# randyjhc/vit-colmap

Hardware: AMD Instinct MI355X
Metric: images/sec extracted + pair-matches/sec (N×D brute-force NN) (higher is better)
Workload: dtype bf16 (ViT) / u8+i32 (matcher); 1 GPU; configs[1]+configs[2]: DINOv2 ViT-S/14 extract of 50 640x480 images (512 keypoints, 384-D uint8 descriptors) then exhaustive mutual-NN + ratio matching of all pairs among the extracted images; images_total=50, images_rank0=50, num_keypoints=512, descriptor_dim=384, parallelism=images+pairs sharded x1

## Files before the change

vit_colmap_amd/csrc/gemm.hip:

```cpp
#include <hip/hip_runtime.h>
#include <stdint.h>

#include "../../include/vitcolmap_hip.h"
#include "common.h"
#include "device.h"

namespace {

typedef __bf16 v8bf __attribute__((ext_vector_type(8)));
typedef __bf16 v4bf __attribute__((ext_vector_type(4)));
typedef float v4f __attribute__((ext_vector_type(4)));

constexpr int BM = 128;
constexpr int BN = 128;
constexpr int BK = 64;
constexpr int kImg = 128 * 128;
constexpr int kStage = 2 * kImg;

enum { EPI_BIAS = 0, EPI_GELU = 1, EPI_RESIDUAL = 2, EPI_PATCH = 3, EPI_SWIGLU = 4 };
static_assert(EPI_BIAS == VC_EPI_BIAS && EPI_GELU == VC_EPI_GELU && EPI_RESIDUAL == VC_EPI_RESIDUAL && EPI_SWIGLU == VC_EPI_SWIGLU,
              "epilogue codes of the ABI");

__device__ __forceinline__ float gelu_erf(float x) {
  const float ax = __builtin_fabsf(x);
// ... 520 lines not shown
        const int row = 8 * p + prow;
        *(v4u*)(tp + row * 128 + (((lane & 7) ^ ((row >> 1) & 7)) << 4)) = *(const v4u*)&xf[4 * c + p];
      }
#pragma unroll
      for (int k4 = 0; k4 < 4; ++k4)
        xf[4 * c + k4] = *(const v8bf*)(tp + r * 128 + (((2 * k4 + h) ^ fsw) << 4));
    }
    if (LN) {
      auto expand = [](uint32_t u) { return (v2f){__uint_as_float(u << 16), __uint_as_float(u & 0xffff0000u)}; };
      v2f s2 = {0.f, 0.f};
#pragma unroll
      for (int ks = 0; ks < XKS; ++ks) {
        const v4u u = *(const v4u*)&xf[ks];
#pragma unroll
        for (int j = 0; j < 4; ++j) s2 += expand(u[j]);
      }
      float sum = s2[0] + s2[1];
      sum += __shfl_xor(sum, 32);
      const float mean = sum * (1.0f / XK);
      const v2f mean2 = {mean, mean};
#pragma unroll
      for (int ks = 0; ks < XKS; ++ks) asm volatile("" : "+v"(xf[ks]));
      v2f q2 = {0.f, 0.f};
#pragma unroll
      for (int ks = 0; ks < XKS; ++ks) {
        const v4u u = *(const v4u*)&xf[ks];
#pragma unroll
        for (int j = 0; j < 4; ++j) { const v2f d = expand(u[j]) - mean2; q2 = __builtin_elementwise_fma(d, d, q2); }
      }
      float q = q2[0] + q2[1];
      q += __shfl_xor(q, 32);
      const float rstd = __builtin_amdgcn_rsqf(q * (1.0f / XK) + eps);
      const v2f rstd2 = {rstd, rstd};
#pragma unroll
      for (int ks = 0; ks < XKS; ++ks) asm volatile("" : "+v"(xf[ks]));
#pragma unroll
      for (int ks = 0; ks < XKS; ++ks) {
        const v4u u = *(const v4u*)&xf[ks];
#pragma unroll
        for (int j = 0; j < 4; ++j) {
          const v2f y = (expand(u[j]) - mean2) * rstd2;
          xf[ks][2 * j] = (__bf16)y[0];
          xf[ks][2 * j + 1] = (__bf16)y[1];
        }
      }
    }
  };

  const __amdgpu_buffer_rsrc_t out_rs = __builtin_amdgcn_make_buffer_rsrc(out, 0, (int)((size_t)M * N * 2), 0x00020000);
  uint8_t* const tr_out = lds + XOffStage + wave * (2 * XChunk);
  uint8_t* const tr_res = tr_out + 2048;
  const int crow = lane >> 2, cch = lane & 3;
  const int rsw = (r >> 2) & 3;
  v4u resq[2];
  auto load_res = [&](int m_base, int nb) {
    if (EPI == EPI_RESIDUAL) {
#pragma unroll
      for (int q = 0; q < 2; ++q)
        resq[q] = *(const v4u*)(res + (size_t)min(m_base + crow + 16 * q, M - 1) * N + nb * 32 + cch * 8);
    }
  };
  v16f pa;
  float ev[16];
  uint32_t ep[8];
  v4u eo[2];
  int pm_base = 0, pnb = 0;
  auto res_to_lds = [&]() {
    if (EPI == EPI_RESIDUAL) {
#pragma unroll
      for (int q = 0; q < 2; ++q) {
        const int row = crow + 16 * q;
        *(v4u*)(tr_res + row * 64 + ((cch ^ ((row >> 2) & 3)) << 4)) = resq[q];
      }
    }
  };
  uint32_t gq[8];
  uint32_t gres[8];
  uint32_t gbad = 0;
  auto slice = [&](int sl) {
    if (EPI == EPI_GELU && GT) {
      typedef __bf16 v2bf __attribute__((ext_vector_type(2)));
      if (sl < 4) {
        const int g = sl;
        const v2bf lo = {(__bf16)pa[4 * g], (__bf16)pa[4 * g + 1]}, hi = {(__bf16)pa[4 * g + 2], (__bf16)pa[4 * g + 3]};
        ep[2 * g] = *(const uint32_t*)&lo;
        ep[2 * g + 1] = *(const uint32_t*)&hi;
        if (sl == 0) gbad = 0;
      }
      if (sl >= 4 && sl < 12) {
        const int qd = sl - 4;
        const uint32_t b0 = ep[qd] & 0xffffu, b1 = ep[qd] >> 16;
        const uint32_t k0 = (b0 & 0x7fffu) - kGtLo, k1 = (b1 & 0x7fffu) - kGtLo;
        gbad = max(gbad, max(k0, k1));
        const uint32_t a0 = min(k0, kGtN - 1) * 4 + ((b0 >> 15) << 1), a1 = min(k1, kGtN - 1) * 4 + ((b1 >> 15) << 1);
        gq[2 * (qd & 3)] = *(const uint16_t*)(gt_l + a0);
        gq[2 * (qd & 3) + 1] = *(const uint16_t*)(gt_l + a1);
      }
      if (sl >= 7 && sl < 15) {
        const int qd = sl - 7;
        gres[qd] = gq[2 * (qd & 3)] | (gq[2 * (qd & 3) + 1] << 16);
      }
      if (sl == 15) {
        if (__any(gbad >= kGtN)) {
#pragma unroll
          for (int qd = 0; qd < 8; ++qd) {
            const v2f_t xin = {__uint_as_float(ep[qd] << 16), __uint_as_float(ep[qd] & 0xffff0000u)};
            const v2f_t y = gelu_erf2(xin);
            const v2bf o = {(__bf16)y[0], (__bf16)y[1]};
            ep[qd] = *(const uint32_t*)&o;
          }
        } else {
#pragma unroll
          for (int qd = 0; qd < 8; ++qd) ep[qd] = gres[qd];
        }
      }
      if (sl == 16) {
#pragma unroll
        for (int i = 0; i < 4; ++i) {
          const auto sw = __builtin_amdgcn_permlane32_swap(ep[i], ep[i + 4], false, false);
          ep[i] = sw[0];
          ep[i + 4] = sw[1];
        }
      }
      if (sl == 17) {
        *(v4u*)(tr_out + r * 64 + (((2 * h) ^ rsw) << 4)) = (v4u){ep[0], ep[1], ep[4], ep[5]};
        *(v4u*)(tr_out + r * 64 + (((2 * h + 1) ^ rsw) << 4)) = (v4u){ep[2], ep[3], ep[6], ep[7]};
      }
      if (sl == 19) {
#pragma unroll
        for (int q = 0; q < 2; ++q) {
          const int row = crow + 16 * q;
          eo[q] = *(const v4u*)(tr_out + row * 64 + ((cch ^ ((row >> 2) & 3)) << 4));
        }
      }
      if (sl == 22) {
#pragma unroll
        for (int q = 0; q < 2; ++q) {
          const int row = crow + 16 * q;
          __builtin_amdgcn_raw_buffer_store_b128(eo[q], out_rs, (int)(((size_t)(pm_base + row) * N + pnb * 32 + cch * 8) * 2), 0, 0);
        }
      }
      return;
    }
    if (sl < 8) {
      const int j0 = 2 * sl;
      if (EPI == EPI_GELU) {
        const v2f_t y = gelu_erf2((v2f_t){pa[j0], pa[j0 + 1]});
        ev[j0] = y[0];
        ev[j0 + 1] = y[1];
      } else if (EPI == EPI_RESIDUAL) {
        if ((sl & 1) == 0) {
          const int g = sl >> 1;
          const v4bf rv = *(const v4bf*)(tr_res + r * 64 + ((g ^ rsw) << 4) + 8 * h);
#pragma unroll
          for (int j = 0; j < 4; ++j) ev[4 * g + j] = pa[4 * g + j] + (float)rv[j];
        }
      } else {
        ev[j0] = pa[j0];
        ev[j0 + 1] = pa[j0 + 1];
      }
    } else if (sl < 12) {
      const int g = sl - 8;
      typedef __bf16 v2bf __attribute__((ext_vector_type(2)));
      const v2bf lo = {(__bf16)ev[4 * g], (__bf16)ev[4 * g + 1]}, hi = {(__bf16)ev[4 * g + 2], (__bf16)ev[4 * g + 3]};
      ep[2 * g] = *(const uint32_t*)&lo;
      ep[2 * g + 1] = *(const uint32_t*)&hi;
    } else if (sl == 12) {
#pragma unroll
      for (int i = 0; i < 4; ++i) {
        const auto sw = __builtin_amdgcn_permlane32_swap(ep[i], ep[i + 4], false, false);
        ep[i] = sw[0];
        ep[i + 4] = sw[1];
      }
    } else if (sl == 13) {
      *(v4u*)(tr_out + r * 64 + (((2 * h) ^ rsw) << 4)) = (v4u){ep[0], ep[1], ep[4], ep[5]};
      *(v4u*)(tr_out + r * 64 + (((2 * h + 1) ^ rsw) << 4)) = (v4u){ep[2], ep[3], ep[6], ep[7]};
    } else if (sl == 15) {
#pragma unroll
      for (int q = 0; q < 2; ++q) {
        const int row = crow + 16 * q;
        eo[q] = *(const v4u*)(tr_out + row * 64 + ((cch ^ ((row >> 2) & 3)) << 4));
      }
    } else if (sl == 19) {
#pragma unroll
      for (int q = 0; q < 2; ++q) {
        const int row = crow + 16 * q;
        __builtin_amdgcn_raw_buffer_store_b128(eo[q], out_rs, (int)(((size_t)(pm_base + row) * N + pnb * 32 + cch * 8) * 2), 0, 0);
      }
    }
  };

  v16f acc;
  int mt_cur = -1, slot = 0;
  int mt = s0 / n_nb, nb = s0 - mt * n_nb;
  for (int i = 0; i < n; ++i) {
    if (i >= 2) {
      if (EPI == EPI_RESIDUAL) asm volatile("s_waitcnt vmcnt(7)" ::: "memory");
      else asm volatile("s_waitcnt vmcnt(5)" ::: "memory");
    } else {
      asm volatile("s_waitcnt vmcnt(3)" ::: "memory");
    }
    asm volatile("s_waitcnt lgkmcnt(0)\n\ts_barrier" ::: "memory");
    const bool pending = i > 0;
    if (pending) res_to_lds();
    const bool reload = mt != mt_cur;
    const int m_base = mt * XRows + wave * 32;
    if (reload) {
      x_issue(mt);
      if (pending) {
#pragma unroll
        for (int sl = 0; sl < XKS; ++sl) slice(sl);
      }
      x_finish();
      mt_cur = mt;
    }
    load_res(m_base, nb);
    const uint8_t* st = lds + slot * XStage + lane * 16;
    {
      const float* bl = bias_l + nb * 32 + 4 * h;
#pragma unroll
      for (int g = 0; g < 4; ++g) {
        const v4f bv = *(const v4f*)(bl + 8 * g);
#pragma unroll
        for (int j = 0; j < 4; ++j) acc[4 * g + j] = bv[j];
      }
    }
    {
      constexpr int XRD = (EPI == EPI_GELU && GT) ? 6 : XReadAhead;
      v8bf wf[XKS];
#pragma unroll
      for (int ks = 0; ks < XRD; ++ks) wf[ks] = *(const v8bf*)(st + ks * 1024);
      __builtin_amdgcn_sched_barrier(0);
      if (pending && !reload) {
#pragma unroll
        for (int ks = 0; ks < XKS; ++ks) {
          acc = __builtin_amdgcn_mfma_f32_32x32x16_bf16(wf[ks], xf[ks], acc, 0, 0, 0);
          if (ks + XRD < XKS) wf[ks + XRD] = *(const v8bf*)(st + (ks + XRD) * 1024);
          slice(ks);
          if (ks == XIssue0 || ks == XIssue0 + XIssueStep || ks == XIssue0 + 2 * XIssueStep)
            issue_piece((ks - XIssue0) / XIssueStep);
          __builtin_amdgcn_sched_barrier(0);
        }
      } else {
#pragma unroll
        for (int ks = 0; ks < XKS; ++ks) {
          acc = __builtin_amdgcn_mfma_f32_32x32x16_bf16(wf[ks], xf[ks], acc, 0, 0, 0);
          if (ks + XRD < XKS) wf[ks + XRD] = *(const v8bf*)(st + (ks + XRD) * 1024);
          if (ks == XIssue0 || ks == XIssue0 + XIssueStep || ks == XIssue0 + 2 * XIssueStep)
            issue_piece((ks - XIssue0) / XIssueStep);
          __builtin_amdgcn_sched_barrier(0);
        }
      }
    }
    pa = acc;
    pm_base = m_base;
    pnb = nb;
    slot = slot + 1 == XNS ? 0 : slot + 1;
    if (++nb == n_nb) { nb = 0; ++mt; }
  }
  res_to_lds();
#pragma unroll
  for (int sl = 0; sl < XKS; ++sl) slice(sl);
  asm volatile("s_waitcnt vmcnt(0)" ::: "memory");
}

__global__ __launch_bounds__(256) void xs_prepare_kernel(const float* __restrict__ W, const float* __restrict__ b,
                                                         const float* __restrict__ gamma, const float* __restrict__ beta,
                                                         int N, __bf16* __restrict__ Wp, float* __restrict__ biasf) {
  const int lane = threadIdx.x & 63;
  const int nfeat = blockIdx.x * 4 + (threadIdx.x >> 6);
  if (nfeat >= N) return;
  const int nb = nfeat >> 5, rr = nfeat & 31;
  float dot = 0.f;
  for (int k = lane; k < XK; k += 64) {
    const float w = W[(size_t)nfeat * XK + k];
    const float wg = gamma ? w * gamma[k] : w;
    if (beta) dot += w * beta[k];
    const int ks = k >> 4, hh = (k >> 3) & 1, j = k & 7;
    Wp[(((size_t)nb * XKS + ks) * 64 + hh * 32 + rr) * 8 + j] = (__bf16)wg;
  }
#pragma unroll
  for (int o = 32; o > 0; o >>= 1) dot += __shfl_xor(dot, o);
  if (lane == 0) biasf[nfeat] = (b ? b[nfeat] : 0.f) + dot;
}


constexpr int MStage = 2 * XStage;
constexpr int MNS = 2;

constexpr int M2OffB1 = MNS * MStage;
constexpr int M2OffGt = M2OffB1 + 1536 * 4;
constexpr int M2OffB2 = M2OffGt + 8704;
constexpr int M2OffTrA = M2OffB2 + 1536;
constexpr int M2OffTrB = M2OffTrA + 4 * XChunk;
constexpr int M2OffG = M2OffTrB + 4 * XChunk;
constexpr int M2Lds = M2OffG + 2 * 4 * 2048;
static_assert(M2Lds <= 160 * 1024, "fused MLP: LDS budget");

constexpr int M2ReadAhead = 6;
constexpr int M2PiecesA = 3;
constexpr int M2Issue0 = 1;
constexpr int M2IssueStep = 3;
constexpr int M2IssueStepB = 2;
__global__ __launch_bounds__(512, 2) void mlp2_kernel(__bf16* __restrict__ X, const uint8_t* __restrict__ Wm,
                                                      const float* __restrict__ b1f, const float* __restrict__ b2f,
                                                      int M, int n_chunks, int n_tiles, float eps,
                                                      const uint16_t* __restrict__ gelu_tab) {
  __shared__ __attribute__((aligned(1024))) uint8_t lds[M2Lds];
  const int tid = threadIdx.x, lane = tid & 63;
  const int wave = __builtin_amdgcn_readfirstlane(tid >> 6);
  const bool roleB = wave >= 4;
  const int pairw = wave & 3;
  const int r = lane & 31, h = lane >> 5;
  const int G = gridDim.x, bid = blockIdx.x;
  const int my_tiles = bid < n_tiles ? (n_tiles - bid + G - 1) / G : 0;
  const int n = my_tiles * n_chunks;
  if (n <= 0) return;

  float* const b1_l = (float*)(lds + M2OffB1);
  float* const b2_l = (float*)(lds + M2OffB2);
  uint8_t* const gt_l = lds + M2OffGt;
  for (int i = tid; i < n_chunks * 32; i += 512) b1_l[i] = b1f[i];
  for (int i = tid; i < XK; i += 512) b2_l[i] = b2f[i];
  for (int i = tid; i < kGtBytes / 4; i += 512) ((uint32_t*)gt_l)[i] = ((const uint32_t*)gelu_tab)[i];

  const uint32_t lds0 = vc::lds_addr(&lds[0]);
  const uint32_t lane_off = (uint32_t)lane * 16u;
  constexpr int NA = M2PiecesA, NB = 12 - NA;
  auto issue_piece = [&](int c1, int c2, int slot, int i) {
    const int role = wave >> 2, q = wave & 3;
    if (i >= (role ? NB : NA)) return;
    const int id = role ? 4 * NA + q * NB + i : q * NA + i;
    const int half = id >= 24, idx = id - 24 * half;
    const int c = half ? c2 : c1;
    const uint8_t* sbase = Wm + (size_t)c * MStage + (size_t)half * XStage + (size_t)idx * 1024;
    const uint32_t dst = lds0 + (uint32_t)slot * MStage + (uint32_t)half * XStage + (uint32_t)idx * 1024u;
    vc::lds_dma16(sbase, lane_off, dst);
  };
  auto issue = [&](int c1, int c2, int slot) {
#pragma unroll
    for (int i = 0; i < (NA > NB ? NA : NB); ++i) issue_piece(c1, c2, slot, i);
  };
  typedef __bf16 v2bf __attribute__((ext_vector_type(2)));
  typedef float v2f __attribute__((ext_vector_type(2)));

  int chunk = 0, slot = 0, tile = bid;
  auto chunk_of = [&](int j) { return j % n_chunks; };
  auto issue_stage = [&](int j, int slot_) {
    const int c1 = chunk_of(min(max(j, 0), n - 1)), c2 = chunk_of(min(max(j - 2, 0), n - 1));
    issue(c1, c2, slot_);
  };
  issue_stage(0, 0);
  if (!roleB) {
    v8bf xf[XKS];
    uint8_t* const tp = lds + M2OffTrA + pairw * XChunk;
    const int prow = lane >> 3;
    v16f hprev;
    uint32_t pb[8], gq[8], gres[8], gbad = 0;
    auto gelu_slice = [&](int sl, int parity) {
      if (sl < 4) {
        const int g = sl;
        const v2bf lo = {(__bf16)hprev[4 * g], (__bf16)hprev[4 * g + 1]}, hi = {(__bf16)hprev[4 * g + 2], (__bf16)hprev[4 * g + 3]};
        pb[2 * g] = *(const uint32_t*)&lo;
        pb[2 * g + 1] = *(const uint32_t*)&hi;
        if (sl == 0) gbad = 0;
      }
      if (sl >= 4 && sl < 12) {
        const int qd = sl - 4;
        const uint32_t b0 = pb[qd] & 0xffffu, b1 = pb[qd] >> 16;
        const uint32_t k0 = (b0 & 0x7fffu) - kGtLo, k1 = (b1 & 0x7fffu) - kGtLo;
        gbad = max(gbad, max(k0, k1));
        gq[2 * (qd & 3)] = *(const uint16_t*)(gt_l + min(k0, kGtN - 1) * 4 + ((b0 >> 15) << 1));
        gq[2 * (qd & 3) + 1] = *(const uint16_t*)(gt_l + min(k1, kGtN - 1) * 4 + ((b1 >> 15) << 1));
      }
      if (sl >= 7 && sl < 15) {
        const int qd = sl - 7;
        gres[qd] = gq[2 * (qd & 3)] | (gq[2 * (qd & 3) + 1] << 16);
      }
      if (sl == 15) {
        if (__any(gbad >= kGtN)) {
#pragma unroll
          for (int qd = 0; qd < 8; ++qd) {
            const v2f_t y = gelu_erf2((v2f_t){__uint_as_float(pb[qd] << 16), __uint_as_float(pb[qd] & 0xffff0000u)});
            const v2bf o = {(__bf16)y[0], (__bf16)y[1]};
            gres[qd] = *(const uint32_t*)&o;
          }
        }
      }
      if (sl == 16) {
        uint8_t* const gb = lds + M2OffG + (parity * 4 + pairw) * 2048 + lane * 16;
        *(v4u*)gb = (v4u){gres[0], gres[1], gres[2], gres[3]};
        *(v4u*)(gb + 1024) = (v4u){gres[4], gres[5], gres[6], gres[7]};
      }
    };
    for (int i = 0; i <= n + 1; ++i) {
      asm volatile("s_waitcnt vmcnt(0)" ::: "memory");
      asm volatile("s_waitcnt lgkmcnt(0)\n\ts_barrier" ::: "memory");
      const bool do_issue = i <= n;
      const int nc1 = chunk_of(min(max(i + 1, 0), n - 1)), nc2 = chunk_of(min(max(i - 1, 0), n - 1));
      if (do_issue && !(i < n && i > 0)) issue_stage(i + 1, slot ^ 1);
      if (i < n) {
        if (chunk == 0) {
          const int m0w = tile * 128 + pairw * 32;
#pragma unroll
          for (int p = 0; p < 4; ++p) {
            const int m = min(m0w + 8 * p + prow, M - 1);
            const uint8_t* src = (const uint8_t*)X + (size_t)m * (XK * 2) + (lane & 7) * 16;
#pragma unroll
            for (int c = 0; c < XK / 64; ++c) *(v4u*)&xf[4 * c + p] = *(const v4u*)(src + c * 128);
          }
          const int fsw = (r >> 1) & 7;
#pragma unroll
          for (int c = 0; c < XK / 64; ++c) {
#pragma unroll
            for (int p = 0; p < 4; ++p) {
              const int row = 8 * p + prow;
              *(v4u*)(tp + row * 128 + (((lane & 7) ^ ((row >> 1) & 7)) << 4)) = *(const v4u*)&xf[4 * c + p];
            }
#pragma unroll
            for (int k4 = 0; k4 < 4; ++k4)
              xf[4 * c + k4] = *(const v8bf*)(tp + r * 128 + (((2 * k4 + h) ^ fsw) << 4));
          }
          auto expand = [](uint32_t u) { return (v2f){__uint_as_float(u << 16), __uint_as_float(u & 0xffff0000u)}; };
          v2f s2 = {0.f, 0.f};
#pragma unroll
          for (int ks = 0; ks < XKS; ++ks) {
            const v4u u = *(const v4u*)&xf[ks];
#pragma unroll
            for (int j = 0; j < 4; ++j) s2 += expand(u[j]);
          }
          float sum = s2[0] + s2[1];
          sum += __shfl_xor(sum, 32);
          const float mean = sum * (1.0f / XK);
          const v2f mean2 = {mean, mean};
#pragma unroll
          for (int ks = 0; ks < XKS; ++ks) asm volatile("" : "+v"(xf[ks]));
          v2f q2 = {0.f, 0.f};
#pragma unroll
          for (int ks = 0; ks < XKS; ++ks) {
            const v4u u = *(const v4u*)&xf[ks];
#pragma unroll
            for (int j = 0; j < 4; ++j) { const v2f d = expand(u[j]) - mean2; q2 = __builtin_elementwise_fma(d, d, q2); }
          }
          float q = q2[0] + q2[1];
          q += __shfl_xor(q, 32);
          const float rstd = __builtin_amdgcn_rsqf(q * (1.0f / XK) + eps);
          const v2f rstd2 = {rstd, rstd};
#pragma unroll
          for (int ks = 0; ks < XKS; ++ks) asm volatile("" : "+v"(xf[ks]));
#pragma unroll
          for (int ks = 0; ks < XKS; ++ks) {
            const v4u u = *(const v4u*)&xf[ks];
#pragma unroll
            for (int j = 0; j < 4; ++j) {
              const v2f y = (expand(u[j]) - mean2) * rstd2;
              xf[ks][2 * j] = (__bf16)y[0];
              xf[ks][2 * j + 1] = (__bf16)y[1];
            }
          }
        }
        const uint8_t* st = lds + slot * MStage + lane * 16;
        v16f hacc;
        {
          const float* bl = b1_l + chunk * 32 + 4 * h;
#pragma unroll
          for (int g = 0; g < 4; ++g) {
            const v4f bv = *(const v4f*)(bl + 8 * g);
#pragma unroll
            for (int j = 0; j < 4; ++j) hacc[4 * g + j] = bv[j];
          }
        }
        {
          constexpr int RD = M2ReadAhead;
          v8bf wf[XKS];
#pragma unroll
          for (int ks = 0; ks < RD; ++ks) wf[ks] = *(const v8bf*)(st + ks * 1024);
          __builtin_amdgcn_sched_barrier(0);
          __builtin_amdgcn_s_setprio(1);
          if (i > 0) {
#pragma unroll
            for (int ks = 0; ks < XKS; ++ks) {
              hacc = __builtin_amdgcn_mfma_f32_32x32x16_bf16(wf[ks], xf[ks], hacc, 0, 0, 0);
              if (ks + RD < XKS) wf[ks + RD] = *(const v8bf*)(st + (ks + RD) * 1024);
              gelu_slice(ks, (i - 1) & 1);
              if (ks >= M2Issue0 && ks < M2Issue0 + NA * M2IssueStep && (ks - M2Issue0) % M2IssueStep == 0 && do_issue)
                issue_piece(nc1, nc2, slot ^ 1, (ks - M2Issue0) / M2IssueStep);
              __builtin_amdgcn_sched_barrier(0);
            }
          } else {
#pragma unroll
            for (int ks = 0; ks < XKS; ++ks) {
              hacc = __builtin_amdgcn_mfma_f32_32x32x16_bf16(wf[ks], xf[ks], hacc, 0, 0, 0);
              if (ks + RD < XKS) wf[ks + RD] = *(const v8bf*)(st + (ks + RD) * 1024);
              __builtin_amdgcn_sched_barrier(0);
            }
          }
        }
        __builtin_amdgcn_s_setprio(0);
        hprev = hacc;
        if (++chunk == n_chunks) { chunk = 0; tile += G; }
      } else if (i == n) {
#pragma unroll
        for (int sl = 0; sl < XKS; ++sl) gelu_slice(sl, (i - 1) & 1);
      }
      slot ^= 1;
    }
  } else {
    v16f oacc[12];
    const __amdgpu_buffer_rsrc_t out_rs = __builtin_amdgcn_make_buffer_rsrc(X, 0, (int)((size_t)M * XK * 2), 0x00020000);
    const int crow = lane >> 2, cch = lane & 3;
    const int rsw = (r >> 2) & 3;
    uint8_t* const tr_out = lds + M2OffTrB + pairw * XChunk;
    uint8_t* const tr_res = tr_out + 2048;
    int pchunk = 0;
    for (int i = 0; i <= n + 1; ++i) {
      asm volatile("s_waitcnt vmcnt(0)" ::: "memory");
      asm volatile("s_waitcnt lgkmcnt(0)\n\ts_barrier" ::: "memory");
      const bool do_issue = i <= n;
      const int nc1 = chunk_of(min(max(i + 1, 0), n - 1)), nc2 = chunk_of(min(max(i - 1, 0), n - 1));
      if (i >= 2) {
        if (pchunk == 0) {
#pragma unroll
          for (int ob = 0; ob < 12; ++ob)
#pragma unroll
            for (int j = 0; j < 16; ++j) oacc[ob][j] = 0.f;
        }
        const uint8_t* gb = lds + M2OffG + ((i & 1) * 4 + pairw) * 2048 + lane * 16;
        const v8bf g_s0 = *(const v8bf*)gb, g_s1 = *(const v8bf*)(gb + 1024);
        const uint8_t* st2 = lds + slot * MStage + XStage + lane * 16;
        {
          constexpr int RD = M2ReadAhead;
          v8bf wf[24];
#pragma unroll
          for (int q = 0; q < RD; ++q) wf[q] = *(const v8bf*)(st2 + q * 1024);
#pragma unroll
          for (int q = 0; q < 24; ++q) {
            oacc[q >> 1] = __builtin_amdgcn_mfma_f32_32x32x16_bf16(wf[q], (q & 1) ? g_s1 : g_s0, oacc[q >> 1], 0, 0, 0);
            if (q + RD < 24) wf[q + RD] = *(const v8bf*)(st2 + (q + RD) * 1024);
            constexpr int BSTEP = NB <= 6 ? M2IssueStep : M2IssueStepB;
            if (q >= M2Issue0 && q < M2Issue0 + NB * BSTEP && (q - M2Issue0) % BSTEP == 0 && do_issue)
              issue_piece(nc1, nc2, slot ^ 1, (q - M2Issue0) / BSTEP);
          }
        }
        if (pchunk == n_chunks - 1) {
          const int m0w = tile * 128 + pairw * 32;
#pragma unroll 1
          for (int ob = 0; ob < 12; ++ob) {
            v4u resq[2];
#pragma unroll
            for (int q = 0; q < 2; ++q)
              resq[q] = *(const v4u*)(X + (size_t)min(m0w + crow + 16 * q, M - 1) * XK + ob * 32 + cch * 8);
#pragma unroll
            for (int q = 0; q < 2; ++q) {
              const int row = crow + 16 * q;
              *(v4u*)(tr_res + row * 64 + ((cch ^ ((row >> 2) & 3)) << 4)) = resq[q];
            }
            v16f oa;
            switch (ob) {
#define VC_OB(k) case k: oa = oacc[k]; break;
              VC_OB(0) VC_OB(1) VC_OB(2) VC_OB(3) VC_OB(4) VC_OB(5) VC_OB(6) VC_OB(7) VC_OB(8) VC_OB(9) VC_OB(10)
              default: oa = oacc[11]; break;
#undef VC_OB
            }
            uint32_t ep[8];
#pragma unroll
            for (int g = 0; g < 4; ++g) {
              const v4bf rv = *(const v4bf*)(tr_res + r * 64 + ((g ^ rsw) << 4) + 8 * h);
              const v4f bv = *(const v4f*)(b2_l + ob * 32 + 8 * g + 4 * h);
              float v[4];
#pragma unroll
              for (int j = 0; j < 4; ++j) v[j] = oa[4 * g + j] + bv[j] + (float)rv[j];
              const v2bf lo = {(__bf16)v[0], (__bf16)v[1]}, hi = {(__bf16)v[2], (__bf16)v[3]};
              ep[2 * g] = *(const uint32_t*)&lo;
              ep[2 * g + 1] = *(const uint32_t*)&hi;
            }
#pragma unroll
            for (int k = 0; k < 4; ++k) {
              const auto sw = __builtin_amdgcn_permlane32_swap(ep[k], ep[k + 4], false, false);
              ep[k] = sw[0];
              ep[k + 4] = sw[1];
            }
            *(v4u*)(tr_out + r * 64 + (((2 * h) ^ rsw) << 4)) = (v4u){ep[0], ep[1], ep[4], ep[5]};
            *(v4u*)(tr_out + r * 64 + (((2 * h + 1) ^ rsw) << 4)) = (v4u){ep[2], ep[3], ep[6], ep[7]};
#pragma unroll
            for (int q = 0; q < 2; ++q) {
              const int row = crow + 16 * q;
              const v4u o = *(const v4u*)(tr_out + row * 64 + ((cch ^ ((row >> 2) & 3)) << 4));
              __builtin_amdgcn_raw_buffer_store_b128(o, out_rs, (int)(((size_t)(m0w + row) * XK + ob * 32 + cch * 8) * 2), 0, 0);
            }
          }
          tile += G;
        }
        if (++pchunk == n_chunks) pchunk = 0;
      }
      if (do_issue && i < 2) issue_stage(i + 1, slot ^ 1);
      slot ^= 1;
    }
  }
}

__global__ __launch_bounds__(256) void mlp_prepare_kernel(const float* __restrict__ W1, const float* __restrict__ b1,
                                                          const float* __restrict__ gamma, const float* __restrict__ beta,
                                                          const float* __restrict__ W2, const float* __restrict__ b2,
                                                          int n_hid, __bf16* __restrict__ Wm, float* __restrict__ b1f,
                                                          float* __restrict__ b2f) {
  const int lane = threadIdx.x & 63;
  const int unit = blockIdx.x * 4 + (threadIdx.x >> 6);
  if (unit < n_hid) {
    const int c = unit >> 5, rr = unit & 31;
    float dot = 0.f;
    for (int k = lane; k < XK; k += 64) {
      const float w = W1[(size_t)unit * XK + k];
      if (beta) dot += w * beta[k];
      const int ks = k >> 4, hh = (k >> 3) & 1, j = k & 7;
      Wm[(size_t)c * (MStage / 2) + ((size_t)ks * 64 + hh * 32 + rr) * 8 + j] = (__bf16)(gamma ? w * gamma[k] : w);
    }
#pragma unroll
    for (int o = 32; o > 0; o >>= 1) dot += __shfl_xor(dot, o);
    if (lane == 0) b1f[unit] = (b1 ? b1[unit] : 0.f) + dot;
  } else if (unit < n_hid + XK) {
    const int f = unit - n_hid, ob = f >> 5, rr = f & 31;
    for (int hd = lane; hd < n_hid; hd += 64) {
      const int c = hd >> 5, e = hd & 31, s = e >> 4, e16 = e & 15;
      const int hh = (e16 >> 2) & 1, j = ((e16 >> 3) << 2) | (e16 & 3);
      Wm[(size_t)c * (MStage / 2) + (XStage / 2) + ((size_t)(2 * ob + s) * 64 + hh * 32 + rr) * 8 + j] = (__bf16)W2[(size_t)f * n_hid + hd];
    }
    if (lane == 0) b2f[f] = b2 ? b2[f] : 0.f;
  }
}

}

static int max_rows_below_2gib(int n_cols, int tile_rows) {
  const long long r = ((1LL << 31) - 1) / ((long long)n_cols * 2);
  return (int)(r / tile_rows * tile_rows);
}

extern "C" {

int vc_linear_bf16(const void* x, const void* weight, const void* bias, const void* residual_or_null, void* out,
                   int rows, int n_out, int k_in, int epilogue, vc_stream_t stream) {
  if (!x || !weight || !bias || !out || rows < 0 || n_out <= 0 || k_in <= 0) return VC_ERR_INVALID_ARG;
  if (epilogue != EPI_BIAS && epilogue != EPI_GELU && epilogue != EPI_RESIDUAL && epilogue != EPI_SWIGLU)
    return VC_ERR_INVALID_ARG;
  if ((epilogue == EPI_RESIDUAL) != (residual_or_null != nullptr)) return VC_ERR_INVALID_ARG;
  if (n_out % (epilogue == EPI_SWIGLU ? 2 * BN : BN) != 0 || k_in % BK != 0) return VC_ERR_UNSUPPORTED;
  if ((((uintptr_t)x) | ((uintptr_t)weight) | ((uintptr_t)bias) | ((uintptr_t)residual_or_null) | ((uintptr_t)out)) % 16 != 0)
    return VC_ERR_INVALID_ARG;
  if (rows == 0) return VC_OK;
  hipStream_t s = (hipStream_t)stream;
  const __bf16 *px = (const __bf16*)x, *pw = (const __bf16*)weight, *pb = (const __bf16*)bias,
               *pr = (const __bf16*)residual_or_null;
  __bf16* po = (__bf16*)out;
  int cus = 0;
  if (int st = vc::cu_count(&cus)) return st;
  if (n_out % G2N == 0 && (long long)((rows + G2M - 1) / G2M) * (n_out / G2N) * 2 >= (long long)cus) {
    const int tiles_m = (rows + G2M - 1) / G2M, tiles_n = n_out / G2N;
    const long long nt = (long long)tiles_m * tiles_n;
    if (nt > 0x7fffffffLL) return VC_ERR_UNSUPPORTED;
    static vc::PerDeviceOnce configured;
    if (int st = vc::allow_dynamic_lds(configured, 160 * 1024, gemm256_kernel<EPI_BIAS, false>, gemm256_kernel<EPI_GELU, false>,
                                       gemm256_kernel<EPI_RESIDUAL, false>, gemm256_kernel<EPI_SWIGLU, false>))
      return st;
    const dim3 grid((unsigned)(nt < cus ? nt : cus)), block(512);
    return vc::dispatch<EPI_BIAS, EPI_GELU, EPI_RESIDUAL, EPI_SWIGLU>(epilogue, [&](auto epi) {
      hipLaunchKernelGGL((gemm256_kernel<epi, false>), grid, block, (size_t)G256_LDS, s, px, pw, pb, pr, po, rows, n_out, k_in,
                         tiles_n, (int)nt, 0, 0, 0, 1, 0, 0, -1);
      return vc::check_launch();
    });
  }
  const int tiles_m = (rows + BM - 1) / BM, tiles_n = n_out / BN;
  const long long nt = (long long)tiles_m * tiles_n;
  if (nt > 0x7fffffffLL) return VC_ERR_UNSUPPORTED;
  return vc::dispatch<EPI_BIAS, EPI_GELU, EPI_RESIDUAL, EPI_SWIGLU>(epilogue, [&](auto epi) {
    hipLaunchKernelGGL(gemm_kernel<epi>, dim3((unsigned)nt), dim3(256), 0, s, px, pw, pb, pr, po, rows, n_out, k_in, tiles_n, (int)nt, 1);
    return vc::check_launch();
  });
}


int vc_conv_taps_bf16(void* x, const void* weight, const void* bias, void* out, int batch, int height, int width, int c_in,
                      int n_out, int kh, int kw, int dy0, int dx0, int out_parity, int epilogue, vc_stream_t stream) {
  if (!x || !weight || !bias || !out || batch < 0 || height <= 0 || width <= 0 || c_in <= 0 || n_out <= 0) return VC_ERR_INVALID_ARG;
  if (epilogue != EPI_BIAS && epilogue != EPI_GELU) return VC_ERR_INVALID_ARG;
  if (kh <= 0 || kw <= 0 || kh * kw > 16 || dy0 < -8 || dy0 > 8 || dx0 < -8 || dx0 > 8) return VC_ERR_INVALID_ARG;
  if (out_parity < -1 || out_parity > 3) return VC_ERR_INVALID_ARG;
  if (n_out % G2N != 0 || c_in % BK != 0) return VC_ERR_UNSUPPORTED;
  if ((((uintptr_t)x) | ((uintptr_t)weight) | ((uintptr_t)bias) | ((uintptr_t)out)) % 16 != 0) return VC_ERR_INVALID_ARG;
  const long long rows = (long long)batch * height * width;
  if (rows == 0) return VC_OK;
  if ((rows + 1 + (long long)(kh + 8) * width) * c_in * 2 >= (1LL << 32) || rows > 0x7fffffffLL) return VC_ERR_UNSUPPORTED;
  hipStream_t s = (hipStream_t)stream;
  if (hipMemsetAsync((char*)x + (size_t)rows * c_in * 2, 0, (size_t)c_in * 2, s) != hipSuccess) return vc::fail(hipGetLastError());
  const int k_total = kh * kw * c_in;
  const int tiles_m = (int)((rows + G2M - 1) / G2M), tiles_n = n_out / G2N;
  const long long nt = (long long)tiles_m * tiles_n;
  if (nt > 0x7fffffffLL) return VC_ERR_UNSUPPORTED;
  static vc::PerDeviceOnce configured;
  if (int st = vc::allow_dynamic_lds(configured, 160 * 1024, gemm256_kernel<EPI_BIAS, true>, gemm256_kernel<EPI_GELU, true>))
    return st;
  int cus = 0;
  if (int st = vc::cu_count(&cus)) return st;
  const dim3 grid((unsigned)(nt < cus ? nt : cus)), block(512);
  const __bf16 *px = (const __bf16*)x, *pw = (const __bf16*)weight, *pb = (const __bf16*)bias;
  __bf16* po = (__bf16*)out;
  return vc::dispatch<EPI_BIAS, EPI_GELU>(epilogue, [&](auto epi) {
    hipLaunchKernelGGL((gemm256_kernel<epi, true>), grid, block, (size_t)G256_LDS, s, px, pw, pb, (const __bf16*)nullptr, po,
                       (int)rows, n_out, k_total, tiles_n, (int)nt, height, width, c_in, kw, dy0, dx0, out_parity);
    return vc::check_launch();
  });
}


size_t vc_linear_xs_weight_bytes(int n_out, int k_in) {
  if (n_out <= 0 || k_in != XK || n_out % 32 != 0) return 0;
  return (size_t)n_out * XK * 2;
}

int vc_linear_xs_prepare(const float* weight, const float* bias_or_null, const float* ln_gamma_or_null,
                         const float* ln_beta_or_null, int n_out, int k_in, void* weight_tiled, float* bias_folded,
                         vc_stream_t stream) {
  if (!weight || !weight_tiled || !bias_folded || n_out <= 0) return VC_ERR_INVALID_ARG;
  if (k_in != XK || n_out % 32 != 0 || n_out > XMaxN) return VC_ERR_UNSUPPORTED;
  if ((ln_gamma_or_null == nullptr) != (ln_beta_or_null == nullptr)) return VC_ERR_INVALID_ARG;
  hipLaunchKernelGGL(xs_prepare_kernel, dim3((n_out + 3) / 4), dim3(256), 0, (hipStream_t)stream, weight, bias_or_null,
                     ln_gamma_or_null, ln_beta_or_null, n_out, (__bf16*)weight_tiled, bias_folded);
  return vc::check_launch();
}

size_t vc_gelu_table_bytes(void) { return (size_t)kGtBytes; }

int vc_gelu_table_bf16(void* table, vc_stream_t stream) {
  if (!table || ((uintptr_t)table) % 16 != 0) return VC_ERR_INVALID_ARG;
  hipLaunchKernelGGL(gelu_table_kernel, dim3((kGtN * 2 + 255) / 256), dim3(256), 0, (hipStream_t)stream, (uint16_t*)table);
  return vc::check_launch();
}

int vc_linear_xs_bf16(const void* x, const void* weight_tiled, const float* bias_folded, const void* residual_or_null,
                      void* out, int rows, int n_out, int k_in, int epilogue, int fuse_layernorm, float ln_eps,
                      const void* gelu_table_or_null, vc_stream_t stream) {
  if (!x || !weight_tiled || !bias_folded || !out || rows < 0 || n_out <= 0) return VC_ERR_INVALID_ARG;
  if (epilogue < EPI_BIAS || epilogue > EPI_RESIDUAL) return VC_ERR_INVALID_ARG;
  if ((epilogue == EPI_RESIDUAL) != (residual_or_null != nullptr)) return VC_ERR_INVALID_ARG;
  if (k_in != XK || n_out % 32 != 0 || n_out > XMaxN) return VC_ERR_UNSUPPORTED;
  if ((((uintptr_t)x) | ((uintptr_t)weight_tiled) | ((uintptr_t)bias_folded) | ((uintptr_t)residual_or_null) | ((uintptr_t)out)) % 16 != 0)
    return VC_ERR_INVALID_ARG;
  if (rows == 0) return VC_OK;
  int cus = 0;
  if (int st = vc::cu_count(&cus)) return st;
  const int n_nb = n_out / 32;
  hipStream_t s = (hipStream_t)stream;
  const uint8_t* pw = (const uint8_t*)weight_tiled;
  const uint16_t* gt = (const uint16_t*)gelu_table_or_null;
  if (gt && (((uintptr_t)gt) % 16 != 0)) return VC_ERR_INVALID_ARG;
  const bool use_gt = gt && epilogue == EPI_GELU && ((n_out * 4 + 15) & ~15) + kGtBytes <= XMaxN * 4;
  const int chunk = max_rows_below_2gib(n_out, XRows);
  for (long long r0 = 0; r0 < rows; r0 += chunk) {
    const int m = (int)(rows - r0 < chunk ? rows - r0 : chunk);
    const int stages = (m + XRows - 1) / XRows * n_nb;
    const dim3 grid((unsigned)(stages < cus ? stages : cus)), block(512);
    const __bf16* px = (const __bf16*)x + (size_t)r0 * XK;
    const __bf16* pr = residual_or_null ? (const __bf16*)residual_or_null + (size_t)r0 * n_out : nullptr;
    __bf16* po = (__bf16*)out + (size_t)r0 * n_out;
    auto launch = [&](auto epi, auto ln, auto gt_on) {
      hipLaunchKernelGGL((xs_kernel<epi, ln, gt_on>), grid, block, 0, s, px, pw, bias_folded, pr, po, m, n_out, n_nb, stages,
                         ln_eps, gt);
      return vc::check_launch();
    };
    const int st = vc::dispatch<EPI_BIAS, EPI_GELU, EPI_RESIDUAL>(epilogue, [&](auto epi) {
      return vc::dispatch<true, false>(fuse_layernorm != 0, [&](auto ln) {
        if constexpr (epi == EPI_GELU) {
          if (use_gt) return launch(epi, ln, std::true_type{});
        }
        return launch(epi, ln, std::false_type{});
      });
    });
    if (st != VC_OK) return st;
  }
  return VC_OK;
}


int vc_patch_embed_bf16(const void* patches, const void* weight, const void* bias, const void* pos_embed, void* out,
                        int n_images, int tokens, int n_out, int k_in, vc_stream_t stream) {
  if (!patches || !weight || !bias || !pos_embed || !out || n_images < 0 || tokens <= 0 || n_out <= 0 || k_in <= 0)
    return VC_ERR_INVALID_ARG;
  if (n_out % BN != 0 || k_in % BK != 0) return VC_ERR_UNSUPPORTED;
  if ((((uintptr_t)patches) | ((uintptr_t)weight) | ((uintptr_t)bias) | ((uintptr_t)pos_embed) | ((uintptr_t)out)) % 16 != 0)
    return VC_ERR_INVALID_ARG;
  if (n_images == 0) return VC_OK;
  const long long rows = (long long)n_images * tokens;
  const long long nt = ((rows + BM - 1) / BM) * (n_out / BN);
  if (rows > 0x7fffffffLL || nt > 0x7fffffffLL) return VC_ERR_UNSUPPORTED;
  hipLaunchKernelGGL(gemm_kernel<EPI_PATCH>, dim3((unsigned)nt), dim3(256), 0, (hipStream_t)stream, (const __bf16*)patches,
                     (const __bf16*)weight, (const __bf16*)bias, (const __bf16*)pos_embed, (__bf16*)out, (int)rows, n_out,
                     k_in, n_out / BN, (int)nt, tokens);
  return vc::check_launch();
}


size_t vc_mlp_weight_bytes(int n_hidden, int dim) {
  if (dim != XK || n_hidden <= 0 || n_hidden % 32 != 0 || n_hidden > 1536) return 0;
  return (size_t)(n_hidden / 32) * MStage;
}

int vc_mlp_prepare(const float* w1, const float* b1_or_null, const float* ln_gamma_or_null, const float* ln_beta_or_null,
                   const float* w2, const float* b2_or_null, int n_hidden, int dim, void* weights_tiled, float* b1_folded,
                   float* b2_out, vc_stream_t stream) {
  if (!w1 || !w2 || !weights_tiled || !b1_folded || !b2_out) return VC_ERR_INVALID_ARG;
  if (vc_mlp_weight_bytes(n_hidden, dim) == 0) return VC_ERR_UNSUPPORTED;
  if ((ln_gamma_or_null == nullptr) != (ln_beta_or_null == nullptr)) return VC_ERR_INVALID_ARG;
  hipLaunchKernelGGL(mlp_prepare_kernel, dim3((n_hidden + XK + 3) / 4), dim3(256), 0, (hipStream_t)stream, w1, b1_or_null,
                     ln_gamma_or_null, ln_beta_or_null, w2, b2_or_null, n_hidden, (__bf16*)weights_tiled, b1_folded, b2_out);
  return vc::check_launch();
}

int vc_mlp_bf16(void* x_inout, const void* weights_tiled, const float* b1_folded, const float* b2, const void* gelu_table,
                int rows, int n_hidden, int dim, float ln_eps, vc_stream_t stream) {
  if (!x_inout || !weights_tiled || !b1_folded || !b2 || !gelu_table || rows < 0) return VC_ERR_INVALID_ARG;
  if (vc_mlp_weight_bytes(n_hidden, dim) == 0) return VC_ERR_UNSUPPORTED;
  if ((((uintptr_t)x_inout) | ((uintptr_t)weights_tiled) | ((uintptr_t)b1_folded) | ((uintptr_t)b2) | ((uintptr_t)gelu_table)) % 16 != 0)
    return VC_ERR_INVALID_ARG;
  if (rows == 0) return VC_OK;
  int cus = 0;
  if (int st = vc::cu_count(&cus)) return st;
  const int chunk = max_rows_below_2gib(XK, 128);
  for (long long r0 = 0; r0 < rows; r0 += chunk) {
    const int m = (int)(rows - r0 < chunk ? rows - r0 : chunk);
    const int n_tiles = (m + 127) / 128;
    const dim3 grid((unsigned)(n_tiles < cus ? n_tiles : cus));
    hipLaunchKernelGGL(mlp2_kernel, grid, dim3(512), 0, (hipStream_t)stream, (__bf16*)x_inout + (size_t)r0 * XK,
                       (const uint8_t*)weights_tiled, b1_folded, b2, m, n_hidden / 32, n_tiles, ln_eps, (const uint16_t*)gelu_table);
    if (int st = vc::check_launch()) return st;
  }
  return VC_OK;
}

}
```

Baseline: 7632 images/s.

## Prefetch MLP residual rows into an LDS ring via DMA during the last chunk

```diff
diff --git a/vit_colmap_amd/csrc/gemm.hip b/vit_colmap_amd/csrc/gemm.hip
--- a/vit_colmap_amd/csrc/gemm.hip
+++ b/vit_colmap_amd/csrc/gemm.hip
@@ -846,6 +846,27 @@
 constexpr int M2Issue0 = 1;
 constexpr int M2IssueStep = 3;
 constexpr int M2IssueStepB = 2;
+constexpr int M2ResDepth = 3;
+static_assert(M2ResDepth >= 1 && M2ResDepth <= 3, "fused MLP: the residual ring has three slots");
+constexpr int m2_res_wait(int ob) {
+  int younger = 0;
+  bool seen = false;
+  for (int b = 0; b < M2ResDepth; ++b) {
+    if (seen) younger += 2;
+    if (b == ob) seen = true;
+  }
+  for (int o = 0; o < 12; ++o) {
+    if (o == ob) return younger;
+    if (o + M2ResDepth < 12) {
+      if (seen) younger += 2;
+      if (o + M2ResDepth == ob) seen = true;
+    }
+    if (seen) younger += 2;
+  }
+  return 0;
+}
+constexpr int m2_res_tail() { return m2_res_wait(11) + 2; }
+static_assert(m2_res_wait(0) == 2 * (M2ResDepth - 1) && m2_res_wait(M2ResDepth) == 4 * M2ResDepth - 2, "fused MLP: epilogue wait counts");
 __global__ __launch_bounds__(512, 2) void mlp2_kernel(__bf16* __restrict__ X, const uint8_t* __restrict__ Wm,
                                                       const float* __restrict__ b1f, const float* __restrict__ b2f,
                                                       int M, int n_chunks, int n_tiles, float eps,
@@ -1056,9 +1077,30 @@
     const int rsw = (r >> 2) & 3;
     uint8_t* const tr_out = lds + M2OffTrB + pairw * XChunk;
     uint8_t* const tr_res = tr_out + 2048;
+    auto ring_off = [](int s) { return s == 0 ? M2OffTrB - M2OffTrA + 2048 : (s - 1) * 2048; };
+    const uint32_t ring_a = lds0 + (uint32_t)(M2OffTrA + pairw * XChunk);
+    auto ring_addr = [&](int s) { return ring_a + (uint32_t)ring_off(s); };
+    auto ring_ptr = [&](int s) { return tr_out + (M2OffTrA - M2OffTrB) + ring_off(s); };
+    uint32_t rvo[2];
+    auto set_res_rows = [&]() {
+      const int m0w = tile * 128 + pairw * 32;
+#pragma unroll
+      for (int q = 0; q < 2; ++q)
+        rvo[q] = (uint32_t)min(m0w + crow + 16 * q, M - 1) * (uint32_t)(XK * 2) + (uint32_t)((cch ^ ((crow >> 2) & 3)) << 4);
+    };
+    set_res_rows();
+    auto res_dma = [&](int ob, uint32_t dst) {
+      const uint8_t* xb = (const uint8_t*)X;
+      asm volatile("" : "+s"(xb));
+      vc::lds_dma16(xb + ob * 64, rvo[0], dst);
+      vc::lds_dma16(xb + ob * 64, rvo[1], dst + 1024u);
+    };
+    bool after_epi = false;
     int pchunk = 0;
     for (int i = 0; i <= n + 1; ++i) {
-      asm volatile("s_waitcnt vmcnt(0)" ::: "memory");
+      if (after_epi) asm volatile("s_waitcnt vmcnt(%0)" ::"n"(m2_res_tail()) : "memory");
+      else asm volatile("s_waitcnt vmcnt(0)" ::: "memory");
+      after_epi = false;
       asm volatile("s_waitcnt lgkmcnt(0)\n\ts_barrier" ::: "memory");
       const bool do_issue = i <= n;
       const int nc1 = chunk_of(min(max(i + 1, 0), n - 1)), nc2 = chunk_of(min(max(i - 1, 0), n - 1));
@@ -1084,36 +1126,40 @@
             constexpr int BSTEP = NB <= 6 ? M2IssueStep : M2IssueStepB;
             if (q >= M2Issue0 && q < M2Issue0 + NB * BSTEP && (q - M2Issue0) % BSTEP == 0 && do_issue)
               issue_piece(nc1, nc2, slot ^ 1, (q - M2Issue0) / BSTEP);
+            constexpr int R0 = 24 - 2 * M2ResDepth;
+            static_assert(M2Issue0 + (NB - 1) * BSTEP < R0, "fused MLP: residual copies are issued behind the stage's pieces");
+            if (q >= R0 && (q - R0) % 2 == 0 && n_chunks >= 2 && pchunk == n_chunks - 1)
+              res_dma((q - R0) / 2, ring_addr(((q - R0) / 2) % M2ResDepth));
           }
         }
         if (pchunk == n_chunks - 1) {
           const int m0w = tile * 128 + pairw * 32;
-#pragma unroll 1
+#pragma unroll
           for (int ob = 0; ob < 12; ++ob) {
-            v4u resq[2];
-#pragma unroll
-            for (int q = 0; q < 2; ++q)
-              resq[q] = *(const v4u*)(X + (size_t)min(m0w + crow + 16 * q, M - 1) * XK + ob * 32 + cch * 8);
-#pragma unroll
-            for (int q = 0; q < 2; ++q) {
-              const int row = crow + 16 * q;
-              *(v4u*)(tr_res + row * 64 + ((cch ^ ((row >> 2) & 3)) << 4)) = resq[q];
-            }
-            v16f oa;
-            switch (ob) {
-#define VC_OB(k) case k: oa = oacc[k]; break;
+            if (n_chunks < 2) {
+              res_dma(ob, ring_addr(0));
+              asm volatile("s_waitcnt vmcnt(0)" ::: "memory");
+            } else switch (ob) {
+#define VC_OB(k) case k: asm volatile("s_waitcnt vmcnt(%0)" ::"n"(m2_res_wait(k)) : "memory"); break;
               VC_OB(0) VC_OB(1) VC_OB(2) VC_OB(3) VC_OB(4) VC_OB(5) VC_OB(6) VC_OB(7) VC_OB(8) VC_OB(9) VC_OB(10)
-              default: oa = oacc[11]; break;
+              default: asm volatile("s_waitcnt vmcnt(%0)" ::"n"(m2_res_wait(11)) : "memory"); break;
 #undef VC_OB
             }
+            const uint8_t* const rs = n_chunks >= 2 ? ring_ptr(ob % M2ResDepth) : tr_res;
+            typedef uint32_t v2u __attribute__((ext_vector_type(2)));
+            v2u rv[4];
+#pragma unroll
+            for (int g = 0; g < 4; ++g) rv[g] = *(const v2u*)(rs + r * 64 + ((g ^ rsw) << 4) + 8 * h);
+            asm volatile("s_waitcnt lgkmcnt(0)" : "+v"(rv[0]), "+v"(rv[1]), "+v"(rv[2]), "+v"(rv[3])::"memory");
+            if (ob + M2ResDepth < 12 && n_chunks >= 2) res_dma(ob + M2ResDepth, ring_addr(ob % M2ResDepth));
             uint32_t ep[8];
 #pragma unroll
             for (int g = 0; g < 4; ++g) {
-              const v4bf rv = *(const v4bf*)(tr_res + r * 64 + ((g ^ rsw) << 4) + 8 * h);
               const v4f bv = *(const v4f*)(b2_l + ob * 32 + 8 * g + 4 * h);
               float v[4];
 #pragma unroll
-              for (int j = 0; j < 4; ++j) v[j] = oa[4 * g + j] + bv[j] + (float)rv[j];
+              for (int j = 0; j < 4; ++j)
+                v[j] = oacc[ob][4 * g + j] + bv[j] + __uint_as_float((j & 1) ? rv[g][j >> 1] & 0xffff0000u : rv[g][j >> 1] << 16);
               const v2bf lo = {(__bf16)v[0], (__bf16)v[1]}, hi = {(__bf16)v[2], (__bf16)v[3]};
               ep[2 * g] = *(const uint32_t*)&lo;
               ep[2 * g + 1] = *(const uint32_t*)&hi;
@@ -1130,10 +1176,12 @@
             for (int q = 0; q < 2; ++q) {
               const int row = crow + 16 * q;
               const v4u o = *(const v4u*)(tr_out + row * 64 + ((cch ^ ((row >> 2) & 3)) << 4));
-              __builtin_amdgcn_raw_buffer_store_b128(o, out_rs, (int)(((size_t)(m0w + row) * XK + ob * 32 + cch * 8) * 2), 0, 0);
+              __builtin_amdgcn_raw_buffer_store_b128(o, out_rs, (int)(((size_t)(m0w + row) * XK + cch * 8) * 2), ob * 64, 0);
             }
           }
           tile += G;
+          set_res_rows();
+          after_epi = n_chunks >= 2;
         }
         if (++pchunk == n_chunks) pchunk = 0;
       }
```

Result: no change. 7640 images/s, median of 2 (+0.1%).
